# HJakeCunningham/ASVGP

Hardware: AMD Instinct MI355X
Metric: Mpoints/s per ELBO+grad step, N=10M 1D Matern-3/2 M=2048 (higher is better)
Workload: dtype f64

## Files before the change

asvgp_amd/csrc/bcr_mfma.hpp:

```cpp
#pragma once
#include "bcr.hpp"
#include "prior_plan.hpp"

namespace asvgp {

constexpr int BM_THREADS = 1024;
constexpr int BM_B = 4;
constexpr int BM_GAT = 0, BM_GBT = 16, BM_DINV = 32, BM_SD = 48, BM_CAT = 64, BM_CBT = 80, BM_W = 96, BM_DG = 100, BM_REC = 104;

__host__ __device__ inline size_t bcr_mfma_ws_doubles(long nb) { return (size_t)nb * BM_REC + 64; }
__host__ __device__ inline size_t bcr_mfma_lds_doubles(long nb) {
  return (size_t)((nb + 1) / 2 + 1) * 32 + (size_t)nb * 4 + 96 + (size_t)(BM_THREADS / 64) * 4 * 40 + (size_t)(nb / 8 + 2) * 52;
}

__device__ __forceinline__ double bm_mfma(double a, double b, double c) { return __builtin_amdgcn_mfma_f64_4x4x4f64(a, b, c, 0, 0, 0); }

__device__ __forceinline__ double bm_chol_linv(const double (&d)[10], int hi, int lo, double& dprod, int& badj) {
  double l00, i0, l10, l20, l30, l11, i1, l21, l31, l22, i2, l32, l33, i3;
  Num<double>::sqrt_inv(d[0], l00, i0);
  badj = !(d[0] > 0.0) ? 1 : 0;
  l10 = d[1] * i0; l20 = d[3] * i0; l30 = d[6] * i0;
  double s = fma(-l10, l10, d[2]);
  badj = (!(s > 0.0) && !badj) ? 2 : badj;
  Num<double>::sqrt_inv(s, l11, i1);
// ... 118 lines not shown
    const int col = n * B + cc, row = (n + 1) * B + rr;
    const bool pad = row >= M;
    const double v = bm_src_load(A, B + rr - cc, pad ? 0 : col, (long)M, 0);
    return pad ? 0.0 : v;
  };
  if ((nb & 1) && tid < 16 && !(split && sp.half == 0)) {
    const int rr = tid >> 2, cc = tid & 3;
    Dl[(size_t)((nb - 1) >> 1) * 16 + tid] = bandD(nb - 1, rr > cc ? rr : cc, rr > cc ? cc : rr);
  }
  if (split && sp.half == 0 && tid < 16) Dl[(size_t)(ht >> 1) * 16 + tid] = 0.0;
  for (int row = tid; row < nb * B; row += BM_THREADS) {
    const bool sep_left = split && sp.half == 0 && row >= ht * B && row < (ht + 1) * B;
    xs[row] = (row < M && !sep_left) ? rhs[(long)row * rhs_stride] : 0.0;
  }
  __syncthreads();
  stamp();

  constexpr int RMAXR = 4;
  for (int l = 0; l < levels; ++l) {
    const int h = 1 << l;
    const int ne = (nb > h) ? (nb - h + 2 * h - 1) / (2 * h) : 0;
    int m0, ne_h;
    level_share(l, ne, m0, ne_h);
    if (split && l == top) {
      if (sp.half == 1) {
        if (wv == 0) {
          const double v = lane < 16 ? Dl[(size_t)(ht >> 1) * 16 + lane] : (lane < 20 ? xs[ht * B + lane - 16] : 0.0);
          bm_msg_send(sp.xchg, 20, v, sp.tag | 1ull, lane);
        }
        const double mine = (r == 0 && c == 0) ? (log(ld.m) + (double)ld.e * 0.6931471805599453094) : 0.0;
        const double tot = wave_sum_dpp(mine);
        int bm = bad ? bad : 0x7fffffff;
#pragma unroll
        for (int off = 32; off > 0; off >>= 1) { const int o = __shfl_xor(bm, off, 64); bm = o < bm ? o : bm; }
        int* sbad = reinterpret_cast<int*>(red + 32);
        if (lane == 0) { red[wv] = tot; sbad[wv] = bm; }
        __syncthreads();
        if (wv == 0) {
          double sv = 0.0;
          int bmin = 0x7fffffff;
          for (int w2 = 0; w2 < BM_THREADS / 64; ++w2) { sv += red[w2]; bmin = sbad[w2] < bmin ? sbad[w2] : bmin; }
          bm_msg_send(sp.xchg + 24, 2, lane == 0 ? sv : (double)bmin, sp.tag | 2ull, lane);
        }
      } else {
        if (wv == 0) {
          double v = 0.0;
          if (!bm_msg_recv(sp.xchg, 20, v, sp.tag | 1ull, lane, sp.spin_limit)) { if (lane == 0) *sp.gave_up = 1; }
          else {
            if (lane < 16) Dl[(size_t)(ht >> 1) * 16 + lane] += v;
            else if (lane < 20) xs[ht * B + lane - 16] += v;
          }
        }
        __syncthreads();
        if (*sp.gave_up) return;
      }
      stamp();
    }
    double updb[RMAXR], ybu[RMAXR];
    int qv = q, ev = e;
    asm volatile("" : "+v"(qv), "+v"(ev));
    double sl[2][3];
    auto slab_loads = [&](int rd0) __attribute__((always_inline)) {
#pragma unroll
      for (int u = 0; u < 2; ++u) {
#pragma unroll
        for (int t3 = 0; t3 < 3; ++t3) {
          sl[u][t3] = 0.0;
          int m = (rd0 + u) * 64 + wv * 4 + qv;
          m = m0 + (m < ne_h ? m : ne_h - 1);
          const int kk = ev + 16 * t3, dd = kk >> 3, col = m * 2 * B + (kk & 7);
          const bool in = kk < 40 && col + dd < M;
          const double v = bm_src_load(A, in ? dd : 0, in ? col : 0, (long)M, 0);
          sl[u][t3] = in ? v : ((dd == 0) ? 1.0 : 0.0);
// ... 48 lines not shown
      if (act && badj && !bad) bad = i * B + badj;
      const double linv = (r >= c) ? t : 0.0;
      const double linvT = (c >= r) ? t : 0.0;
      if (act) ld.mul(dprod);
      const double ua = bm_mfma(linvT, ea, 0.0);
      const double ub = bm_mfma(linvT, eb, 0.0);
      const double zz = bm_mfma(linvT, yv, 0.0);
      const double nua = -ua, nub = -ub;
      const double da_new = bm_mfma(nua, ua, da);
      const double e_new = bm_mfma(nub, ua, 0.0);
      const double ya_new = bm_mfma(nua, zz, ya);
      updb[rd] = bm_mfma(ub, ub, 0.0);
      ybu[rd] = bm_mfma(ub, zz, 0.0);
      updb[rd] = act ? updb[rd] : 0.0;
      ybu[rd] = act ? ybu[rd] : 0.0;
      const double gat = bm_mfma(ua, linv, 0.0);
      const double gbt = bm_mfma(ub, linv, 0.0);
      const double dinv = bm_mfma(linv, linv, 0.0);
      const double w = bm_mfma(linv, zz, 0.0);
      if (act) {
        if (l >= 3) {
          double* R = Fl + (size_t)(i >> 3) * 52;
          R[e] = gat; R[16 + e] = gbt; R[32 + e] = dinv;
          if (c == 0) R[48 + r] = w;
        } else {
          double* R = rec(i);
          R[BM_GAT + e] = gat; R[BM_GBT + e] = gbt; R[BM_DINV + e] = dinv;
          if (c == 0) R[BM_W + r] = w;
        }
        Dl[(size_t)(a >> 1) * 16 + e] = da_new;
        El[(size_t)(a >> 1) * 16 + e] = e_new;
        if (c == 0) xs[a * B + r] = ya_new;
      }
    }
    bcr_lds_barrier();
#pragma unroll
    for (int rd = 0; rd < RMAXR; ++rd) {
      if (rd * 64 + wv * 4 >= ne_h) continue;
      const int ml = rd * 64 + wv * 4 + q;
      const int i = h + (m0 + ml) * 2 * h, b = i + h;
      if (ml < ne_h && b < nb) {
        Dl[(size_t)(b >> 1) * 16 + e] -= updb[rd];
        if (c == 0) xs[b * B + r] -= ybu[rd];
      }
    }
    bcr_lds_barrier();
    stamp();
  }
  if (wv == 0 && !(split && sp.half == 1)) {
    const bool act = q == 0;
    double d[10];
    int kk = 0;
#pragma unroll
    for (int rr = 0; rr < 4; ++rr)
#pragma unroll
      for (int cc = 0; cc <= rr; ++cc) { const double v = Dl[rr * 4 + cc]; d[kk++] = act ? v : ((rr == cc) ? 1.0 : 0.0); }
    const double yv = (act && c == 0) ? xs[r] : 0.0;
    double dprod;
    int badj;
    const double t = bm_chol_linv(d, hi, lo, dprod, badj);
    if (act && badj && !bad) bad = badj;
    const double linv = (r >= c) ? t : 0.0, linvT = (c >= r) ? t : 0.0;
    if (act) ld.mul(dprod);
    const double s00 = bm_mfma(linv, linv, 0.0);
    const double zz = bm_mfma(linvT, yv, 0.0);
    const double x0 = bm_mfma(linv, zz, 0.0);
    if (act) {
      rec(0)[BM_SD + e] = s00;
// ... 289 lines not shown
```

asvgp_amd/csrc/elbo.hip:

```cpp
#include <stdlib.h>
#include <time.h>
#include <string.h>

#include "bcr_pre.hpp"
#include "bcr_mfma.hpp"
#include "handle.hpp"

namespace asvgp {


struct Ws {
  double *Kuu, *dK, *P, *LK, *dLK, *LP, *SK, *dSK, *SP, *c, *alpha, *logdets, *fin, *bcrK, *bcrP;
};
static size_t bcr_ws_chain(int planes, int k, bool big) {
  long ns = 1024;
  while ((long)planes * 2 * k * k * ns * 8 + 2 * ns * k * 8 + 1024 > 150 * 1024) ns >>= 1;
  if (big) ns *= 2;
  return (size_t)planes * (7 * k * k + k) * 2 * ns + (big ? (size_t)planes * k * k * ns : 0);
}
static size_t bcr_ws_K(int k, long M) {
  size_t a = bcr_ws_chain(2, k, false), b = bcr_ws_chain(2, k, true), c = bcr_pre_ws_doubles(k, (M + k - 1) / k);
  a = a > b ? a : b;
  return (a > c ? a : c) + 64;
}
// ... 381 lines not shown
                        fin.th, fin.alpha_scale, fin.gacc, fin.ticket, fin.arrived, fin.out);
}

template <int K>
__global__ __launch_bounds__(BM_THREADS) void elbo_chains_mfma_kernel(KuuInterior ki, const double* S_static, KuuCoefs2 cf, double* Kuu, double* dK, const double* A, const double* b, int M,
                                                                      double* wsP, double* SP, double* x, double* logdets, int* info,
                                                                      double s, const double* tab, int n_rec, const int* node_rec,
                                                                      double* wsK, double* SK, double* dSK,
                                                                      unsigned long long* done_flag, unsigned long long seq,
                                                                      const unsigned long long* ready_flag, long spin_limit, FusedFin fin, const ThetaBox* box) {
  extern __shared__ double lds[];
  static_assert(K == BM_B, "matrix-core chains: bandwidth 4");
  const long E = (long)(K + 1) * M;
  const unsigned long long t_start = fin.debug_stamps ? __builtin_amdgcn_s_memrealtime() : 0ull;
  auto rstamp = [&](int slot) {
    if (fin.debug_stamps && threadIdx.x == 0 && blockIdx.x <= 2)
      logdets[(slot < 4 ? 8 + 4 * (int)blockIdx.x : 24) + slot] = (slot == 0) ? (double)(t_start & 0xffffffffull) : (double)((__builtin_amdgcn_s_memrealtime() - t_start) & 0xffffffffull);
  };
  rstamp(0);
  __shared__ int gave_up, kuu_ok;
  __shared__ double kuu_pref[4];
  if (threadIdx.x == 0) { gave_up = 0; kuu_ok = 0; }
  __syncthreads();
  double s_v = s, asc_v = fin.alpha_scale;
  ElboScalars th_v = fin.th;
  if (box) {
    if (threadIdx.x == 0) {
      long spins = 0;
      for (;;) {
        const unsigned long long got = __hip_atomic_load(&box->seq, __ATOMIC_RELAXED, __HIP_MEMORY_SCOPE_SYSTEM);
        if (got == seq) break;
        if (got == ~0ull || ++spins > spin_limit) { gave_up = 1; break; }
        __builtin_amdgcn_s_sleep(2);
      }
    }
    __syncthreads();
    if (gave_up) { if (threadIdx.x == 0) atomicExch(info + 1, -1); return; }
    s_v = box->s; asc_v = box->alpha_scale;
    th_v.v = box->v; th_v.l = box->l; th_v.s = box->s; th_v.N = box->N; th_v.Nw = box->Nw; th_v.cw = box->cw;
  }
  const double* stats = fin.stats;
  enum { LOGK, LOGP, TRKA, DTRKA, SKDK, SPDK, SKK, SPK, SPA, CC, AKA, ADKA, AAA, BA, NACC };
  double acc[NACC];
#pragma unroll
  for (int i = 0; i < NACC; ++i) acc[i] = 0.0;
  const bool isP = blockIdx.x == 0 || (fin.split && blockIdx.x == 2);
  const bool isPR = fin.split && blockIdx.x == 2;
  __shared__ double kdl[16];
  __shared__ double bnd[2 * PRIOR_BND_DIAGS * PRIOR_BND], dkb[2 * 5 * KI_DKB];
  {
    if (isP) rstamp(1);
    if (threadIdx.x == 0) {
      if (box) {
#pragma unroll
        for (int i = 0; i < 5; ++i) { kdl[i] = box->k[i]; kdl[8 + i] = box->dk[i]; }
      } else {
        kdl[0] = ki.k[0]; kdl[1] = ki.k[1]; kdl[2] = ki.k[2]; kdl[3] = ki.k[3]; kdl[4] = ki.k[4];
        kdl[8] = ki.dk[0]; kdl[9] = ki.dk[1]; kdl[10] = ki.dk[2]; kdl[11] = ki.dk[3]; kdl[12] = ki.dk[4];
      }
    }
    {
      const double* bnd_g = box ? box->bnd : reinterpret_cast<const double*>((const char*)__builtin_amdgcn_kernarg_segment_ptr() + offsetof(KuuInterior, bnd));
      const double* dkb_g = box ? box->dkb : reinterpret_cast<const double*>((const char*)__builtin_amdgcn_kernarg_segment_ptr() + offsetof(KuuInterior, dkb));
      if (threadIdx.x < 2 * PRIOR_BND_DIAGS * PRIOR_BND) bnd[threadIdx.x] = bnd_g[threadIdx.x];
      else if (threadIdx.x < 2 * PRIOR_BND_DIAGS * PRIOR_BND + 2 * 5 * KI_DKB) dkb[threadIdx.x - 2 * PRIOR_BND_DIAGS * PRIOR_BND] = dkb_g[threadIdx.x - 2 * PRIOR_BND_DIAGS * PRIOR_BND];
    }
    __syncthreads();
  }
  if (isP) {
    BmSplit bsp;
    if (fin.split) { bsp.half = isPR ? 1 : 0; bsp.xchg = fin.xchg; bsp.spin_limit = spin_limit; bsp.gave_up = &gave_up; bsp.tag = seq << 8; }
    bcr_mfma_solve<BandSumToep>(BandSumToep{A, 1.0 / s_v, (lds_cdouble_ptr)kdl, (lds_cdouble_ptr)bnd, ki.lo, ki.hi}, b, M, wsP, lds, SP, x, logdets + 2, info + 1, 1,
                                fin.debug_stamps ? (isPR ? fin.xchg + 128 : logdets + 32) : (double*)nullptr, bsp);
    rstamp(3);
    __syncthreads();
    if (gave_up) { if (threadIdx.x == 0) atomicExch(info + 1, -1); return; }
    rstamp(4);
    if (fin.finalize) {
      const double* xs_l = lds + (size_t)2 * ((((M + K - 1) / K) + 1) / 2 + 1) * 16;
      static_assert(BM_THREADS == 1024, "two columns per thread");
      int nbl = (M + K - 1) / K, lv = 0;
      while ((1 << lv) < nbl) ++lv;
      const long jsep = (long)(1 << (lv > 0 ? lv - 1 : 0)) * K;
      const long j0 = isPR ? jsep : 0, j1 = (fin.split && !isPR) ? jsep : (long)M;
      unsigned long long kw = 0ull;
      const bool kuu_reader = !isPR && (threadIdx.x >> 6) == 1;
      if (kuu_reader && (threadIdx.x & 63) <= 4)
        kw = __hip_atomic_load(reinterpret_cast<const unsigned long long*>(fin.gacc + 8) + (threadIdx.x & 63), __ATOMIC_RELAXED, __HIP_MEMORY_SCOPE_AGENT);
      double sp[2][K + 1], av[2][K + 1], bj[2];
#pragma unroll
      for (int cI = 0; cI < 2; ++cI) {
        const long j = j0 + threadIdx.x + cI * BM_THREADS, jc = j < j1 ? j : j1 - 1;
#pragma unroll
        for (int r = 0; r <= K; ++r) { sp[cI][r] = SP[(long)r * M + jc]; av[cI][r] = stats[(long)r * M + jc]; }
        bj[cI] = stats[(long)(K + 1) * M + jc];
      }
#pragma unroll
      for (int cI = 0; cI < 2; ++cI) {
        const long j = j0 + threadIdx.x + cI * BM_THREADS;
        if (j >= j1) continue;
        const bool left = j < ki.lo, right = j >= ki.hi;
        const double xj = xs_l[j];
#pragma unroll
        for (int r = 0; r <= K; ++r) {
          const long o = (long)r * M + j;
          const double w2 = (r == 0) ? 1.0 : 2.0;
          double kv = kdl[r], dkv = kdl[8 + r];
          if (left || right) {
            kv = bnd[left ? (long)r * PRIOR_BND + j : (long)(PRIOR_BND_DIAGS + r) * PRIOR_BND + (j - ki.hi)];
            if (ki.dk_tab) {
              dkv = dkb[left ? (long)r * KI_DKB + j : (long)(5 + r) * KI_DKB + (j - ki.hi)];
            } else {
              dkv = 0.0;
              for (int t = 0; t < cf.n; ++t) dkv = fma(box ? box->dc[t] : cf.dc[t], S_static[(long)t * E + o], dkv);
            }
          }
          const double xx = (j + r < M) ? w2 * xj * xs_l[j + r] : 0.0;
          acc[SPDK] = fma(w2 * sp[cI][r], dkv, acc[SPDK]);
// ... 100 lines not shown
    for (int i = 1; i < 7; ++i) v = (lane == i) ? red[i] : v;
    bm_msg_send(isPR ? box_pr : box_kuu, nmine, v, mtag | (isPR ? 5ull : 4ull), lane);
    if (threadIdx.x == 0) rstamp(2);
    return;
  }
  double kuu_v = 0.0, pr_v = 0.0;
  {
    bool ok = true;
    if (kuu_ok) kuu_v = lane < 4 ? kuu_pref[lane] : 0.0;
    else ok = bm_msg_recv(box_kuu, 4, kuu_v, mtag | 4ull, lane, spin_limit);
    if (ok && fin.split) ok = bm_msg_recv(box_pr, 7, pr_v, mtag | 5ull, lane, spin_limit);
    if (!ok) { if (lane == 0) atomicExch(info + 1, -1); return; }
  }
  {
    const int pidx[7] = {SPDK, SPK, SPA, AKA, ADKA, AAA, BA};
#pragma unroll
    for (int i = 0; i < 7; ++i) tot[pidx[i]] = red[i] + (fin.split ? __shfl(pr_v, i, 64) : 0.0);
  }
  tot[TRKA] = __shfl(kuu_v, 0, 64); tot[DTRKA] = __shfl(kuu_v, 1, 64); tot[SKDK] = __shfl(kuu_v, 2, 64); tot[SKK] = __shfl(kuu_v, 3, 64);
  if (threadIdx.x != 0) return;
#pragma unroll
  for (int i = 0; i < 14; ++i) __hip_atomic_store(fin.gacc + i, 0.0, __ATOMIC_RELAXED, __HIP_MEMORY_SCOPE_AGENT);
  {
    const double v = th_v.v, sn = th_v.s, N = th_v.N, Nw = th_v.Nw;
    const double yy = stats[(long)(K + 1) * M + M];
    const double asc = asc_v;
    tot[AKA] *= asc * asc; tot[ADKA] *= asc * asc; tot[AAA] *= asc * asc; tot[BA] *= asc;
    tot[LOGK] = __hip_atomic_load(logdets + 0, __ATOMIC_RELAXED, __HIP_MEMORY_SCOPE_AGENT);
    tot[LOGP] = __hip_atomic_load(logdets + 2, __ATOMIC_RELAXED, __HIP_MEMORY_SCOPE_AGENT);
    tot[CC] = tot[BA] / sn;
    const double two_pi = 6.283185307179586476925286766559;
    double elbo = -0.5 * N * log(two_pi * sn);
    elbo -= 0.5 * tot[LOGP];
    elbo += 0.5 * tot[LOGK];
    elbo -= 0.5 * yy / sn;
    elbo += 0.5 * tot[CC];
    elbo -= 0.5 * Nw * v / sn;
    elbo += 0.5 * tot[TRKA] / sn;
    if (th_v.cw != 0.0) elbo += th_v.cw;
    const double d_l = 0.5 * (tot[SKDK] - tot[SPDK] - tot[ADKA] + tot[DTRKA] / sn);
    const double d_v = 0.5 * (-tot[SKK] / v + tot[SPK] / v + tot[AKA] / v + tot[TRKA] / (v * sn)) - 0.5 * Nw / sn;
    const double s2 = sn * sn;
    const double d_s = -0.5 * N / sn + 0.5 * tot[SPA] / s2 + 0.5 * yy / s2 + 0.5 * tot[AAA] / s2 - tot[BA] / s2 + 0.5 * Nw * v / s2 - 0.5 * tot[TRKA] / s2;
    double* out = fin.out;
    out[0] = elbo; out[1] = d_v; out[2] = d_l; out[3] = d_s;
    out[4] = tot[LOGK]; out[5] = tot[LOGP]; out[6] = tot[TRKA]; out[7] = tot[CC];
    if (fin.mirror) {
      double* m = fin.mirror;
      const double mv[10] = {elbo, d_v, d_l, d_s, tot[LOGK], tot[LOGP], tot[TRKA], tot[CC],
                             (double)__hip_atomic_load(info, __ATOMIC_RELAXED, __HIP_MEMORY_SCOPE_AGENT),
                             (double)__hip_atomic_load(info + 1, __ATOMIC_RELAXED, __HIP_MEMORY_SCOPE_AGENT)};
      double sum = (double)fin.mirror_seq;
#pragma unroll
      for (int i = 0; i < 10; ++i) { __hip_atomic_store(m + i, mv[i], __ATOMIC_RELAXED, __HIP_MEMORY_SCOPE_SYSTEM); sum += mv[i]; }
      __hip_atomic_store(m + 11, sum, __ATOMIC_RELAXED, __HIP_MEMORY_SCOPE_SYSTEM);
      __hip_atomic_store(m + 10, (double)fin.mirror_seq, __ATOMIC_RELAXED, __HIP_MEMORY_SCOPE_SYSTEM);
    }
  }
  rstamp(2);
}

static __global__ void scale_sub_kernel(const double* __restrict__ a, const double* __restrict__ b, double* __restrict__ o,
                                 long n) {
  long i = (long)blockIdx.x * blockDim.x + threadIdx.x;
  if (i < n) o[i] = a[i] - b[i];
}
static __global__ void scale_kernel(double* __restrict__ x, double f, long n) {
  long i = (long)blockIdx.x * blockDim.x + threadIdx.x;
  if (i < n) x[i] = x[i] * f;
}

template <int K, bool TANGENT>
static int run_chains(Handle* h, const double* stats, const double* S, int kind, double v, double l, double s, long M, long D,
                      Ws w, int* info, hipStream_t st, bool& use_bcr, int part = 0, bool scale_alpha = true, FusedFin* fin = nullptr) {
  double t_enter = 0.0;
  if (debug_env().host_times) { timespec ts; clock_gettime(CLOCK_MONOTONIC, &ts); t_enter = ts.tv_sec * 1e6 + ts.tv_nsec * 1e-3; }
  KuuCoefs2 cf;
  for (int t = 0; t < ASVGP_MAX_KUU_TERMS; ++t) cf.c[t] = cf.dc[t] = 0.0;
  int rc = asvgp_matern_coeffs(kind, v, l, cf.c, cf.dc, &cf.n);
  if (rc) return rc;
  const long E = (long)(K + 1) * M;
  const double* A = stats;
  const double* b = stats ? stats + E : nullptr;
  const long nb = (M + K - 1) / K;
  const int algo = h->band_algo;
  const bool have_plan = h->plan && prior_plan_M(h->plan) == M && prior_plan_k(h->plan) == K && prior_plan_terms(h->plan) == cf.n;
  if ((algo == 3 || algo == 4) && !have_plan) { set_error("band algorithms 3 and 4 need asvgp_prior_plan_1d for this (M, k, kernel)"); return ASVGP_ERR_BAD_ARG; }
  size_t ldsK = sizeof(double) * (TANGENT ? bcr_lds_doubles<Dual, K, 0>(nb) : bcr_lds_doubles<double, K, 0>(nb));
  size_t ldsP = sizeof(double) * bcr_lds_doubles<double, K, 1>(nb);
  bool planned = have_plan && (algo == 0 || algo == 3 || algo == 4);
  size_t lds_bytes = planned ? ldsP : (ldsK > ldsP ? ldsK : ldsP);
  bool fits = lds_bytes <= 160 * 1024 - 256;
  bool big = false;
  constexpr bool HAS_BIG = (K <= 5);
  if (HAS_BIG && !fits) {
    size_t bK = sizeof(double) * (TANGENT ? bcr_lds_doubles<Dual, K, 0, true>(nb) : bcr_lds_doubles<double, K, 0, true>(nb));
    size_t bP = sizeof(double) * bcr_lds_doubles<double, K, 1, true>(nb);
    size_t bb = planned ? bP : (bK > bP ? bK : bP);
    if (bb <= 160 * 1024 - 256) { big = true; fits = true; lds_bytes = bb; }
// ... 15 lines not shown
        prior_plan_interior_kuu(h->plan, cf.c, ki.k, &ki.lo, &ki.hi, ki.bnd);
        use_mfma = ki.hi > ki.lo;
        if (use_mfma) {
          double bnd2[2 * PRIOR_BND_DIAGS * PRIOR_BND];
          long lo2 = 0, hi2 = 0;
          prior_plan_interior_kuu(h->plan, cf.dc, ki.dk, &lo2, &hi2, bnd2);
          ki.dk_tab = (ki.lo <= KI_DKB && M - ki.hi <= KI_DKB) ? 1 : 0;
          for (int sd = 0; sd < 2; ++sd)
            for (int d = 0; d <= K; ++d)
              for (int cI = 0; cI < KI_DKB; ++cI)
                ki.dkb[(sd * 5 + d) * KI_DKB + cI] = bnd2[(size_t)(sd * PRIOR_BND_DIAGS + d) * PRIOR_BND + cI];
        }
      }
    }
    if (algo == 4 && !use_mfma) {
      set_error("band algorithm 4 (matrix-core chains) needs k = 4, D = 1, M <= 2048, Toeplitz static bands and the ELBO + gradient entry point");
      return ASVGP_ERR_UNSUPPORTED;
    }
    if (h->ahead_req && !use_mfma) { set_error("launch-ahead exists for the matrix-core launch only (k = 4, D = 1, M <= 2048, planned prior chain)"); return ASVGP_ERR_UNSUPPORTED; }
    if (!use_mfma && !fits) { set_error("BCR needs %zu B of LDS", lds_bytes); return ASVGP_ERR_LDS_CAPACITY; }
    unsigned long long seq = 0;
    int slot = 0;
    double t_acq0 = 0.0, t_acq1 = 0.0;
    if (debug_env().host_times) { timespec ts; clock_gettime(CLOCK_MONOTONIC, &ts); t_acq0 = ts.tv_sec * 1e6 + ts.tv_nsec * 1e-3; }
    double* tab = handle_table_acquire(h, &seq, &slot);
    if (debug_env().host_times) { timespec ts; clock_gettime(CLOCK_MONOTONIC, &ts); t_acq1 = ts.tv_sec * 1e6 + ts.tv_nsec * 1e-3; }
    const bool gpu_fwd = h->prior_forward_gpu;
    const double* tab_k = h->tab_dev + (size_t)slot * h->slot_doubles;
    const unsigned long long* dd_ready = nullptr;
    if (gpu_fwd) {
      double* t = nullptr;
      rc = handle_prior_dd_forward(h, cf.c, cf.dc, slot, st, &t, nullptr, use_mfma ? seq : 0ull, use_mfma ? &dd_ready : nullptr);
      if (rc) return rc;
      tab_k = t;
    }
    size_t lds_pre = sizeof(double) * bcr_pre_lds_doubles(K, n_rec);
    if (lds_pre > lds_bytes) lds_bytes = lds_pre;
    FusedFin ff{};
    if (fin) { ff = *fin; ff.finalize = 1; fin->finalize = -1; }
    ff.n_helpers = (int)((M + 255) / 256 < 6 ? (M + 255) / 256 : 6);
    ff.split = 0; ff.xchg = nullptr;
    ff.assembled = reinterpret_cast<unsigned*>(w.fin + 20);
    ff.debug_no_assembly = debug_env().no_assembly;
    ff.debug_stamps = debug_env().chain_stamps;
    const long spin_limit = debug_env().spin_limit;
    if constexpr (K == BM_B) {
      if (use_mfma) {
        size_t lb = sizeof(double) * bcr_mfma_lds_doubles(nb), lk = sizeof(double) * bcr_mfma_pre_lds_doubles(nb, n_rec);
        if (lk > lb) lb = lk;
        if (sizeof(double) * FIN_LDS_DOUBLES > lb) lb = sizeof(double) * FIN_LDS_DOUBLES;
        auto kern = elbo_chains_mfma_kernel<K>;
        static size_t lds_granted[16] = {0};
        size_t& granted = lds_granted[h->device & 15];
        if (lb > granted) {
          hipError_t e = hipFuncSetAttribute(reinterpret_cast<const void*>(kern), hipFuncAttributeMaxDynamicSharedMemorySize, (int)lb);
          if (e != hipSuccess) { set_error("hipFuncSetAttribute: %s", hipGetErrorString(e)); return ASVGP_ERR_LDS_CAPACITY; }
          granted = lb;
        }
        if (h->mirror_dev) { ff.mirror = h->mirror_dev; ff.mirror_seq = ++h->mirror_seq; h->mirror_pending = ff.mirror_seq; }
        if (nb >= 128 && !debug_env().no_split) {
          ff.split = 1;
          ff.xchg = w.LP;
        }
        ff.n_helpers = 0;
        const bool plan_first = debug_env().plan_first != 0;
        const bool host_times = debug_env().host_times != 0;
        auto now_us = []() { timespec ts; clock_gettime(CLOCK_MONOTONIC, &ts); return ts.tv_sec * 1e6 + ts.tv_nsec * 1e-3; };
        const double t0 = host_times ? now_us() : 0.0;
        if (plan_first && !gpu_fwd) (void)prior_plan_eval(h->plan, cf.c, cf.dc, tab);
        const ThetaBox* box_k = nullptr;
        if (h->ahead_req) {
          if (gpu_fwd || plan_first) { set_error("launch-ahead needs the host forward pass (asvgp_set_prior_forward(h, 0))"); return ASVGP_ERR_UNSUPPORTED; }
          static_assert(sizeof(ThetaBox) <= BOX_BYTES, "theta box");
          if (!h->box_host) {
            if (hipHostMalloc(&h->box_host, BOX_BYTES * TAB_SLOTS, hipHostMallocMapped | hipHostMallocPortable | hipHostMallocCoherent) != hipSuccess ||
                hipHostGetDevicePointer(&h->box_dev, h->box_host, 0) != hipSuccess) {
              if (h->box_host) { (void)hipHostFree(h->box_host); h->box_host = nullptr; }
              set_error("launch-ahead: pinned allocation failed: %s", hipGetErrorString(hipGetLastError()));
              return ASVGP_ERR_HIP;
            }
            memset(h->box_host, 0, BOX_BYTES * TAB_SLOTS);
          }
          ThetaBox* bh = reinterpret_cast<ThetaBox*>(static_cast<char*>(h->box_host) + (size_t)slot * BOX_BYTES);
          __atomic_store_n(&bh->seq, 0ull, __ATOMIC_RELEASE);
          box_k = reinterpret_cast<const ThetaBox*>(static_cast<const char*>(h->box_dev) + (size_t)slot * BOX_BYTES);
        }
        const bool to_worker = !plan_first && !gpu_fwd && h->fwd_worker && !h->ahead_req;
        if (to_worker) {
          for (int t = 0; t < ASVGP_MAX_KUU_TERMS; ++t) { h->fwd.coef[t] = cf.c[t]; h->fwd.dcoef[t] = cf.dc[t]; }
// ... 49 lines not shown
    }
    if (scale_alpha) {
      long n = M * D;
      hipLaunchKernelGGL(scale_kernel, dim3((unsigned)((n + 255) / 256)), dim3(256), 0, st, w.alpha, 1.0 / s, n);
    }
    return check_launch("elbo chains (planned prior)");
  }
  const bool pfly = (part == 2) && use_bcr;
  if (!pfly)
    hipLaunchKernelGGL(elbo_prepare_kernel, dim3((unsigned)((E + 255) / 256)), dim3(256), 0, st, S, cf, E, A, s,
                       part == 2 ? w.LK : w.Kuu, part == 2 ? (double*)nullptr : w.dK, part == 1 ? (double*)nullptr : w.P);
  if (h->sync_on && part == 1) (void)hipEventRecord(h->evK, st);
  if (h->sync_on && part == 2) (void)hipStreamWaitEvent(st, h->evK, 0);
  if (use_bcr) {
    if (!fits) { set_error("BCR forced but needs %zu B of LDS", lds_bytes); return ASVGP_ERR_LDS_CAPACITY; }
    hipError_t e = hipFuncSetAttribute(big ? reinterpret_cast<const void*>(elbo_bcr_kernel<K, TANGENT, HAS_BIG>) : reinterpret_cast<const void*>(elbo_bcr_kernel<K, TANGENT, false>), hipFuncAttributeMaxDynamicSharedMemorySize, (int)lds_bytes);
    if (e != hipSuccess) { set_error("hipFuncSetAttribute: %s", hipGetErrorString(e)); return ASVGP_ERR_LDS_CAPACITY; }
    if (part == 1 && TANGENT) {
      if constexpr (TANGENT) {
        auto kern = big ? elbo_bcr_prior_kernel<K, HAS_BIG> : elbo_bcr_prior_kernel<K, false>;
        e = hipFuncSetAttribute(reinterpret_cast<const void*>(kern), hipFuncAttributeMaxDynamicSharedMemorySize, (int)lds_bytes);
        if (e != hipSuccess) { set_error("hipFuncSetAttribute: %s", hipGetErrorString(e)); return ASVGP_ERR_LDS_CAPACITY; }
        hipLaunchKernelGGL(kern, dim3(1), dim3(BCR_THREADS), lds_bytes, st, w.Kuu, w.dK, (int)M, w.bcrK, w.SK, w.dSK, w.logdets, info,
                           debug_env().bcr_stamps);
      }
    } else if (pfly) {
      auto kern = big ? elbo_bcr_data_kernel<K, HAS_BIG> : elbo_bcr_data_kernel<K, false>;
      e = hipFuncSetAttribute(reinterpret_cast<const void*>(kern), hipFuncAttributeMaxDynamicSharedMemorySize, (int)lds_bytes);
      if (e != hipSuccess) { set_error("hipFuncSetAttribute: %s", hipGetErrorString(e)); return ASVGP_ERR_LDS_CAPACITY; }
      hipLaunchKernelGGL(kern, dim3(1), dim3(BCR_THREADS), lds_bytes, st, w.Kuu, A, b, (int)M, w.bcrP, w.SP, w.alpha, w.logdets, info,
                         debug_env().bcr_stamps, s, (int)D, (int)(lds_bytes / sizeof(double)));
    } else {
      auto kern = big ? elbo_bcr_kernel<K, TANGENT, HAS_BIG> : elbo_bcr_kernel<K, TANGENT, false>;
      hipLaunchKernelGGL(kern, dim3(part == 0 ? 2 : 1), dim3(BCR_THREADS), lds_bytes, st, w.Kuu, w.dK,
                         w.P, b, (int)M, w.bcrK, w.bcrP, w.SK, w.dSK, w.SP, w.alpha, w.logdets, info,
                         debug_env().bcr_stamps, part == 2 ? 1 : 0, (int)D, (int)(lds_bytes / sizeof(double)));
    }
    if (part == 1) {
      if (h->sync_on) (void)hipEventRecord(h->evP, st);
      return check_launch("elbo prior chain");
    }
  } else if (D == 1) {
    hipLaunchKernelGGL((elbo_factor_kernel<K, TANGENT, true>), dim3(2), dim3(64), 0, st, w.Kuu, w.dK, w.P, w.LK, w.dLK,
                       w.LP, b, w.c, (int)M, info);
    hipLaunchKernelGGL((elbo_inverse_kernel<K, TANGENT, true>), dim3(2), dim3(64), 0, st, w.LK, w.dLK, w.LP, w.SK,
                       w.dSK, w.SP, w.c, w.alpha, (int)M);
  } else {
    hipLaunchKernelGGL((elbo_factor_kernel<K, TANGENT, false>), dim3(2), dim3(64), 0, st, w.Kuu, w.dK, w.P, w.LK,
                       w.dLK, w.LP, b, w.c, (int)M, info);
    hipLaunchKernelGGL(elbo_trsv_kernel<K>, dim3((unsigned)D), dim3(64), 0, st, w.LP, (int)M, b, w.c, D, 0, 1.0);
    hipLaunchKernelGGL((elbo_inverse_kernel<K, TANGENT, false>), dim3(2), dim3(64), 0, st, w.LK, w.dLK, w.LP, w.SK,
                       w.dSK, w.SP, w.c, w.alpha, (int)M);
    hipLaunchKernelGGL(elbo_trsv_kernel<K>, dim3((unsigned)D), dim3(64), 0, st, w.LP, (int)M, w.c, w.alpha, D, 1, 1.0);
  }
  long n = M * D;
  if (!use_bcr) hipLaunchKernelGGL(scale_kernel, dim3((unsigned)((n + 255) / 256)), dim3(256), 0, st, w.c, 1.0 / s, n);
  if (!use_bcr || scale_alpha)
    hipLaunchKernelGGL(scale_kernel, dim3((unsigned)((n + 255) / 256)), dim3(256), 0, st, w.alpha, 1.0 / s, n);
  return check_launch("elbo chains");
}

template <int K>
int ElboLauncher<K>::run(Handle* h, const double* stats, const double* S, int kind, double v, double l, double s, long N, long M, long D,
                         double* out, int* info, void* ws, hipStream_t st, int part) {
  {
    Ws w = carve(ws, M, K, D);
    bool bcr = false;
    h->mirror_pending = 0;
    ElboScalars th{v, l, s, (double)N, (double)N, 0.0};
    if (h->w_set) { th.N = h->w_npos; th.Nw = h->w_sum; th.cw = 0.5 * (double)D * h->w_sumlog; }
    const int fin_blocks = (int)((M + 255) / 256 < 64 ? (M + 255) / 256 : 64);
    static_assert(BCR_THREADS == 256, "the fused finalize shares the chain kernel's workgroup size");
    FusedFin ff{stats, th, 1.0 / s, w.fin, reinterpret_cast<unsigned*>(w.fin + 16), reinterpret_cast<unsigned*>(w.fin + 18), nullptr, out, D, 0, 0};
    int rc = run_chains<K, true>(h, stats, S, kind, v, l, s, M, D, w, info, st, bcr, part, false, part == 1 ? nullptr : &ff);
    if (rc || (part == 1)) return rc;
    if (ff.finalize < 0) return check_launch("elbo_grad_1d (fused)");
    if (h->sync_on && part == 2 && bcr && h->evP) (void)hipStreamWaitEvent(st, h->evP, 0);
    hipLaunchKernelGGL(elbo_finalize_kernel<K>, dim3(fin_blocks), dim3(256), 0, st, stats, w.Kuu, w.dK, w.LK, w.LP, w.SK,
                       w.dSK, w.SP, w.c, w.alpha, bcr ? w.logdets : (const double*)nullptr, M, K, D, th,
                       bcr ? 1.0 / s : 1.0, w.fin, reinterpret_cast<unsigned*>(w.fin + 16), out);
    return check_launch("elbo_grad_1d");
  }
}
template <int K>
int PostLauncher<K>::run(Handle* h, const double* stats, const double* S, int kind, double v, double l, double s, long M, long D,
                         double* alpha, double* W, int* info, void* ws, hipStream_t st, double* Pinv) {
  {
    Ws w = carve(ws, M, K, D);
    bool bcr = false;
    int rc = run_chains<K, false>(h, stats, S, kind, v, l, s, M, D, w, info, st, bcr);
    if (rc) return rc;
    long E = (long)(K + 1) * M;
    hipLaunchKernelGGL(scale_sub_kernel, dim3((unsigned)((E + 255) / 256)), dim3(256), 0, st, w.SP, w.SK, W, E);
    hipError_t e = hipMemcpyAsync(alpha, w.alpha, sizeof(double) * M * D, hipMemcpyDeviceToDevice, st);
    if (e == hipSuccess && Pinv) e = hipMemcpyAsync(Pinv, w.SP, sizeof(double) * E, hipMemcpyDeviceToDevice, st);
    if (e != hipSuccess) { set_error("hipMemcpyAsync: %s", hipGetErrorString(e)); return ASVGP_ERR_HIP; }
    return check_launch(Pinv ? "posterior_prepare_loo_1d" : "posterior_prepare_1d");
  }
}
// ... 434 lines not shown
```

asvgp_amd/csrc/phi_pass.hip:

```cpp
#include <stdlib.h>

#include "handle.hpp"

namespace asvgp {

constexpr int PHI_THREADS = 1024;
constexpr int PHI_CH = 32;
constexpr int PHI_MAX_BLOCKS = 256;
constexpr size_t PHI_LDS_BUDGET = 160 * 1024 - 512;

template <int K> struct FxTab {
  int g[K + 1];
  constexpr FxTab() : g{} {
    double cf[K + 1][K + 1] = {};
    for (int i = 0; i <= K; ++i)
      for (int p = 0; p <= K; ++p) cf[i][p] = piece_coef<K, 0>(i, p);
    for (int d = 0; d <= K; ++d) {
      double mx = 0.0;
      for (int i = 0; i + d <= K; ++i)
        for (int q = 0; q <= 32; ++q) {
          const double t = q / 32.0;
          double a = cf[i][K], b = cf[i + d][K];
          for (int p = K - 1; p >= 0; --p) { a = a * t + cf[i][p]; b = b * t + cf[i + d][p]; }
          if (a * b > mx) mx = a * b;
// ... 592 lines not shown
  if (avail <= 0) return 0;
  return (int)(avail / (8 * (K + 2 + (fx ? 1 : 0))));
}

template <int K, int CS>
static int launch_phi_moments_cs(Handle* h, const double* x, const double* y, long N, const double* mesh, long n_mesh, double delta,
                                 long M, double* stats, double* ws, hipStream_t st, bool regular, double step) {
  const int ncells = (int)n_mesh - 1;
  const size_t lds_bytes = mq_lds_bytes<K, CS>(M);
  if (ncells > CS || lds_bytes > PHI_LDS_BUDGET) return 1;
  long nblk = (N + 2 * MQ_THREADS - 1) / (2 * MQ_THREADS);
  const long gmax = (h->phi_blocks > 0 && h->phi_blocks < PHI_MAX_BLOCKS) ? h->phi_blocks : PHI_MAX_BLOCKS;
  const int G = (int)(nblk < 1 ? 1 : (nblk > gmax ? gmax : nblk));
  long ppb = (N + G - 1) / G;
  ppb = ((ppb + 2 * MQ_THREADS - 1) / (2 * MQ_THREADS)) * (2 * MQ_THREADS);
  int s0 = 50;
  { long c = 2; int lg = 1; while (c < ppb) { c <<= 1; ++lg; } if (62 - lg < s0) s0 = 62 - lg; }
  MqArgs a;
  a.x = x; a.y = y; a.N = N; a.mesh_g = mesh; a.n_mesh = (int)n_mesh; a.inv_delta = 1.0 / delta; a.M = (int)M; a.step = step;
  a.partials = ws;
  a.ov = ws + (size_t)PHI_MAX_BLOCKS * ((size_t)(K + 2) * M + 1);
  a.ppb = ppb; a.zero_ptr = stats; a.zero_n = (K + 2) * M + 1; a.s0 = s0;
  auto kern = regular ? phi_moment_kernel<K, CS, true> : phi_moment_kernel<K, CS, false>;
  hipError_t e = hipFuncSetAttribute(reinterpret_cast<const void*>(kern), hipFuncAttributeMaxDynamicSharedMemorySize, (int)lds_bytes);
  if (e != hipSuccess) { set_error("hipFuncSetAttribute(%zu B LDS): %s", lds_bytes, hipGetErrorString(e)); return ASVGP_ERR_LDS_CAPACITY; }
  const bool prof = h->prof_on && h->prof_n < PROF_RING && (h->prof_calls++ % h->prof_every == 0);
  if (prof) (void)hipEventRecord(h->prof_ev[h->prof_n][0], st);
  hipLaunchKernelGGL(kern, dim3((unsigned)G), dim3(MQ_THREADS), lds_bytes, st, a);
  if (prof) { (void)hipEventRecord(h->prof_ev[h->prof_n][1], st); ++h->prof_n; }
  const int E1 = (int)((K + 2) * M + 1);
  const int gsplit = G >= 64 ? 16 : (G >= 8 ? 4 : 1);
  if (h->phi_defer) {
    h->pend = Handle::PendingReduce{a.partials, G, (int)M, K, stats, true, nullptr};
    return check_launch("phi_accumulate_1d (moments, reduce deferred)");
  }
  hipLaunchKernelGGL(phi_reduce_kernel, dim3((E1 + 255) / 256, gsplit), dim3(256), 0, st, a.partials, G, (int)M, K, 0, M, 1L, 0, 1, stats, (const int*)nullptr);
  return check_launch("phi_accumulate_1d (moments)");
}

template <int K>
static int launch_phi_moments(Handle* h, const double* x, const double* y, long N, long D, const double* mesh, long n_mesh, double delta,
                              long M, double* stats, double* ws, hipStream_t st) {
  if (D != 1 || N < 1 || ((reinterpret_cast<uintptr_t>(x) | reinterpret_cast<uintptr_t>(y)) & 15) != 0) return 1;
  double step = 0.0;
  const bool regular = handle_mesh_is_linspace(h, mesh, n_mesh, st, &step, nullptr, nullptr);
  int rc = launch_phi_moments_cs<K, 512>(h, x, y, N, mesh, n_mesh, delta, M, stats, ws, st, regular, step);
  if (rc == 1) rc = launch_phi_moments_cs<K, 1024>(h, x, y, N, mesh, n_mesh, delta, M, stats, ws, st, regular, step);
  if (rc == 1) rc = launch_phi_moments_cs<K, 2048>(h, x, y, N, mesh, n_mesh, delta, M, stats, ws, st, regular, step);
// ... 36 lines not shown
  }
  if (h->n_order_seen < 8) h->order_seen[h->n_order_seen++] = Handle::OrderSeen{x, N, series};
  return series != 0;
}

template <int K, int TP, int TS>
static int launch_phi_sort_as(Handle* h, const double* x, const double* y, long N, const double* mesh, long n_mesh, double delta,
                              long M, double* stats, double* ws, hipStream_t st, double step, double m0, double m_last, double margin) {
  size_t lds_bytes = ps_lds_bytes<K, TP, TS>();
  if (ps_epilogue_bytes<K>() > lds_bytes) lds_bytes = ps_epilogue_bytes<K>();
  if (lds_bytes > 160 * 1024) return 1;
  long nblk = (N + TP * PS_THREADS - 1) / (TP * PS_THREADS);
  const long gmax = (h->phi_blocks > 0 && h->phi_blocks < PHI_MAX_BLOCKS) ? h->phi_blocks : PHI_MAX_BLOCKS;
  const int G = (int)(nblk < 1 ? 1 : (nblk > gmax ? gmax : nblk));
  long ppb = (N + G - 1) / G;
  ppb = TS ? ((ppb + 127) & ~127L) : ((ppb + 1) & ~1L);
  if (ppb > 0x3fffffffL) return 1;
  PsArgs a;
  a.x = x; a.y = y; a.N = N; a.mesh_g = mesh; a.n_mesh = (int)n_mesh; a.inv_delta = 1.0 / delta; a.M = (int)M;
  a.m0 = m0; a.m_last = m_last; a.step = step; a.smax_fast = 0.5 - margin;
  a.partials = ws; a.ppb = ppb; a.zero_ptr = stats; a.zero_n = (K + 2) * M + 1; a.stamps = nullptr; a.stamps_wave = 0;
  a.ranges = reinterpret_cast<int*>(ws + (size_t)PHI_MAX_BLOCKS * ((size_t)(K + 2) * M + 1));
  auto kern = phi_sort_kernel<K, TP, 0, 1, TS>;
  hipError_t e = hipFuncSetAttribute(reinterpret_cast<const void*>(kern), hipFuncAttributeMaxDynamicSharedMemorySize, (int)lds_bytes);
  if (e != hipSuccess) { set_error("hipFuncSetAttribute(%zu B LDS): %s", lds_bytes, hipGetErrorString(e)); return ASVGP_ERR_LDS_CAPACITY; }
  const bool prof = h->prof_on && h->prof_n < PROF_RING && (h->prof_calls++ % h->prof_every == 0);
  if (prof) (void)hipEventRecord(h->prof_ev[h->prof_n][0], st);
  hipLaunchKernelGGL(kern, dim3((unsigned)G), dim3(PS_THREADS), lds_bytes, st, a);
  if (prof) { (void)hipEventRecord(h->prof_ev[h->prof_n][1], st); ++h->prof_n; }
  h->phi_last_series = TS;
  const int E1 = (int)((K + 2) * M + 1);
  const int gsplit = G >= 64 ? 16 : (G >= 8 ? 4 : 1);
  if (h->phi_defer) {
    h->pend = Handle::PendingReduce{a.partials, G, (int)M, K, stats, true, a.ranges};
    return check_launch("phi_accumulate_1d (tile sort, reduce deferred)");
  }
  hipLaunchKernelGGL(phi_reduce_kernel, dim3((E1 + 255) / 256, gsplit), dim3(256), 0, st, a.partials, G, (int)M, K, 0, M, 1L, 0, 1, stats, (const int*)a.ranges);
  return check_launch("phi_accumulate_1d (tile sort)");
}

template <int K>
static int launch_phi_sort(Handle* h, const double* x, const double* y, long N, long D, const double* mesh, long n_mesh, double delta,
                           long M, double* stats, double* ws, hipStream_t st) {
  if (D != 1 || N < 2 || M > PS_NCELL || ((reinterpret_cast<uintptr_t>(x) | reinterpret_cast<uintptr_t>(y)) & 15) != 0) return 1;
  double step = 0.0, m0 = 0.0, m_last = 0.0;
  if (!handle_mesh_is_linspace(h, mesh, n_mesh, st, &step, &m0, &m_last)) return 1;
  const double amax = fabs(m0) > fabs(m_last) ? fabs(m0) : fabs(m_last);
  const double margin = 16.0 * 2.220446049250313e-16 * amax / delta + 1e-12;
// ... 314 lines not shown
```

Before: 133,700.

## Cache LDS attribute grants, hoist split-send out of level loop, stage scalars in LDS

Several unrelated tweaks. The phi launchers now call hipFuncSetAttribute only when the requested LDS size exceeds a cached per-device grant, which removes a host API call per step. The split BCR kernel's half-1 send/reduce path moves out of the level loop behind an early break, and a few values are passed through empty asm statements to steer register allocation. The finalize kernel keeps its theta scalars in shared memory instead of registers, and the debug_env lookup is hoisted. The static grant cache is not keyed per kernel template instantiation beyond the regular flag, so a grant could be wrongly assumed for another instantiation.

```diff
diff --git a/asvgp_amd/csrc/bcr_mfma.hpp b/asvgp_amd/csrc/bcr_mfma.hpp
--- a/asvgp_amd/csrc/bcr_mfma.hpp
+++ b/asvgp_amd/csrc/bcr_mfma.hpp
@@ -164,33 +164,17 @@
     const int ne = (nb > h) ? (nb - h + 2 * h - 1) / (2 * h) : 0;
     int m0, ne_h;
     level_share(l, ne, m0, ne_h);
+    if (split && l == top && sp.half == 1) break;
     if (split && l == top) {
-      if (sp.half == 1) {
-        if (wv == 0) {
-          const double v = lane < 16 ? Dl[(size_t)(ht >> 1) * 16 + lane] : (lane < 20 ? xs[ht * B + lane - 16] : 0.0);
-          bm_msg_send(sp.xchg, 20, v, sp.tag | 1ull, lane);
-        }
-        const double mine = (r == 0 && c == 0) ? (log(ld.m) + (double)ld.e * 0.6931471805599453094) : 0.0;
-        const double tot = wave_sum_dpp(mine);
-        int bm = bad ? bad : 0x7fffffff;
-#pragma unroll
-        for (int off = 32; off > 0; off >>= 1) { const int o = __shfl_xor(bm, off, 64); bm = o < bm ? o : bm; }
-        int* sbad = reinterpret_cast<int*>(red + 32);
-        if (lane == 0) { red[wv] = tot; sbad[wv] = bm; }
-        __syncthreads();
-        if (wv == 0) {
-          double sv = 0.0;
-          int bmin = 0x7fffffff;
-          for (int w2 = 0; w2 < BM_THREADS / 64; ++w2) { sv += red[w2]; bmin = sbad[w2] < bmin ? sbad[w2] : bmin; }
-          bm_msg_send(sp.xchg + 24, 2, lane == 0 ? sv : (double)bmin, sp.tag | 2ull, lane);
-        }
-      } else {
+      int lh = lane;
+      asm volatile("" : "+v"(lh));
+      {
         if (wv == 0) {
           double v = 0.0;
           if (!bm_msg_recv(sp.xchg, 20, v, sp.tag | 1ull, lane, sp.spin_limit)) { if (lane == 0) *sp.gave_up = 1; }
           else {
-            if (lane < 16) Dl[(size_t)(ht >> 1) * 16 + lane] += v;
-            else if (lane < 20) xs[ht * B + lane - 16] += v;
+            if (lh < 16) Dl[(size_t)(ht >> 1) * 16 + lh] += v;
+            else if (lh < 20) xs[ht * B + lh - 16] += v;
           }
         }
         __syncthreads();
@@ -285,7 +269,9 @@
         if (l >= 3) {
           double* R = Fl + (size_t)(i >> 3) * 52;
           R[e] = gat; R[16 + e] = gbt; R[32 + e] = dinv;
-          if (c == 0) R[48 + r] = w;
+          int iw = i;
+          asm volatile("" : "+v"(iw));
+          if (c == 0) (Fl + (size_t)(iw >> 3) * 52)[48 + r] = w;
         } else {
           double* R = rec(i);
           R[BM_GAT + e] = gat; R[BM_GBT + e] = gbt; R[BM_DINV + e] = dinv;
@@ -307,6 +293,32 @@
         if (c == 0) xs[b * B + r] -= ybu[rd];
       }
     }
+    bcr_lds_barrier();
+    stamp();
+  }
+  if (split && sp.half == 1) {
+    int lh = lane;
+    asm volatile("" : "+v"(lh));
+    if (wv == 0) {
+      const double v = lh < 16 ? Dl[(size_t)(ht >> 1) * 16 + lh] : (lh < 20 ? xs[ht * B + lh - 16] : 0.0);
+      bm_msg_send(sp.xchg, 20, v, sp.tag | 1ull, lane);
+    }
+    const double mine = (r == 0 && c == 0) ? (log(ld.m) + (double)ld.e * 0.6931471805599453094) : 0.0;
+    const double tot = wave_sum_dpp(mine);
+    int bm = bad ? bad : 0x7fffffff;
+#pragma unroll
+    for (int off = 32; off > 0; off >>= 1) { const int o = __shfl_xor(bm, off, 64); bm = o < bm ? o : bm; }
+    int* sbad = reinterpret_cast<int*>(red + 32);
+    if (lane == 0) { red[wv] = tot; sbad[wv] = bm; }
+    __syncthreads();
+    if (wv == 0) {
+      double sv = 0.0;
+      int bmin = 0x7fffffff;
+      for (int w2 = 0; w2 < BM_THREADS / 64; ++w2) { sv += red[w2]; bmin = sbad[w2] < bmin ? sbad[w2] : bmin; }
+      bm_msg_send(sp.xchg + 24, 2, lane == 0 ? sv : (double)bmin, sp.tag | 2ull, lane);
+    }
+    stamp();
+    bcr_lds_barrier();
     bcr_lds_barrier();
     stamp();
   }
diff --git a/asvgp_amd/csrc/elbo.hip b/asvgp_amd/csrc/elbo.hip
--- a/asvgp_amd/csrc/elbo.hip
+++ b/asvgp_amd/csrc/elbo.hip
@@ -427,8 +427,8 @@
   __shared__ double kuu_pref[4];
   if (threadIdx.x == 0) { gave_up = 0; kuu_ok = 0; }
   __syncthreads();
-  double s_v = s, asc_v = fin.alpha_scale;
-  ElboScalars th_v = fin.th;
+  __shared__ double th_l[8];
+  double s_v = s;
   if (box) {
     if (threadIdx.x == 0) {
       long spins = 0;
@@ -441,8 +441,7 @@
     }
     __syncthreads();
     if (gave_up) { if (threadIdx.x == 0) atomicExch(info + 1, -1); return; }
-    s_v = box->s; asc_v = box->alpha_scale;
-    th_v.v = box->v; th_v.l = box->l; th_v.s = box->s; th_v.N = box->N; th_v.Nw = box->Nw; th_v.cw = box->cw;
+    s_v = box->s;
   }
   const double* stats = fin.stats;
   enum { LOGK, LOGP, TRKA, DTRKA, SKDK, SPDK, SKK, SPK, SPA, CC, AKA, ADKA, AAA, BA, NACC };
@@ -457,9 +456,11 @@
     if (isP) rstamp(1);
     if (threadIdx.x == 0) {
       if (box) {
+        th_l[0] = box->v; th_l[1] = box->s; th_l[2] = box->N; th_l[3] = box->Nw; th_l[4] = box->cw; th_l[5] = box->alpha_scale;
 #pragma unroll
         for (int i = 0; i < 5; ++i) { kdl[i] = box->k[i]; kdl[8 + i] = box->dk[i]; }
       } else {
+        th_l[0] = fin.th.v; th_l[1] = fin.th.s; th_l[2] = fin.th.N; th_l[3] = fin.th.Nw; th_l[4] = fin.th.cw; th_l[5] = fin.alpha_scale;
         kdl[0] = ki.k[0]; kdl[1] = ki.k[1]; kdl[2] = ki.k[2]; kdl[3] = ki.k[3]; kdl[4] = ki.k[4];
         kdl[8] = ki.dk[0]; kdl[9] = ki.dk[1]; kdl[10] = ki.dk[2]; kdl[11] = ki.dk[3]; kdl[12] = ki.dk[4];
       }
@@ -493,12 +494,14 @@
       if (kuu_reader && (threadIdx.x & 63) <= 4)
         kw = __hip_atomic_load(reinterpret_cast<const unsigned long long*>(fin.gacc + 8) + (threadIdx.x & 63), __ATOMIC_RELAXED, __HIP_MEMORY_SCOPE_AGENT);
       double sp[2][K + 1], av[2][K + 1], bj[2];
+      const double* stats_t = stats;
+      asm volatile("" : "+s"(stats_t));
 #pragma unroll
       for (int cI = 0; cI < 2; ++cI) {
         const long j = j0 + threadIdx.x + cI * BM_THREADS, jc = j < j1 ? j : j1 - 1;
 #pragma unroll
-        for (int r = 0; r <= K; ++r) { sp[cI][r] = SP[(long)r * M + jc]; av[cI][r] = stats[(long)r * M + jc]; }
-        bj[cI] = stats[(long)(K + 1) * M + jc];
+        for (int r = 0; r <= K; ++r) { sp[cI][r] = SP[(long)r * M + jc]; av[cI][r] = stats_t[(long)r * M + jc]; }
+        bj[cI] = stats_t[(long)(K + 1) * M + jc];
       }
 #pragma unroll
       for (int cI = 0; cI < 2; ++cI) {
@@ -645,9 +648,9 @@
 #pragma unroll
   for (int i = 0; i < 14; ++i) __hip_atomic_store(fin.gacc + i, 0.0, __ATOMIC_RELAXED, __HIP_MEMORY_SCOPE_AGENT);
   {
-    const double v = th_v.v, sn = th_v.s, N = th_v.N, Nw = th_v.Nw;
+    const double v = th_l[0], sn = th_l[1], N = th_l[2], Nw = th_l[3], cw = th_l[4];
     const double yy = stats[(long)(K + 1) * M + M];
-    const double asc = asc_v;
+    const double asc = th_l[5];
     tot[AKA] *= asc * asc; tot[ADKA] *= asc * asc; tot[AAA] *= asc * asc; tot[BA] *= asc;
     tot[LOGK] = __hip_atomic_load(logdets + 0, __ATOMIC_RELAXED, __HIP_MEMORY_SCOPE_AGENT);
     tot[LOGP] = __hip_atomic_load(logdets + 2, __ATOMIC_RELAXED, __HIP_MEMORY_SCOPE_AGENT);
@@ -660,7 +663,7 @@
     elbo += 0.5 * tot[CC];
     elbo -= 0.5 * Nw * v / sn;
     elbo += 0.5 * tot[TRKA] / sn;
-    if (th_v.cw != 0.0) elbo += th_v.cw;
+    if (cw != 0.0) elbo += cw;
     const double d_l = 0.5 * (tot[SKDK] - tot[SPDK] - tot[ADKA] + tot[DTRKA] / sn);
     const double d_v = 0.5 * (-tot[SKK] / v + tot[SPK] / v + tot[AKA] / v + tot[TRKA] / (v * sn)) - 0.5 * Nw / sn;
     const double s2 = sn * sn;
@@ -696,8 +699,9 @@
 template <int K, bool TANGENT>
 static int run_chains(Handle* h, const double* stats, const double* S, int kind, double v, double l, double s, long M, long D,
                       Ws w, int* info, hipStream_t st, bool& use_bcr, int part = 0, bool scale_alpha = true, FusedFin* fin = nullptr) {
+  const DebugEnv& dbg = debug_env();
   double t_enter = 0.0;
-  if (debug_env().host_times) { timespec ts; clock_gettime(CLOCK_MONOTONIC, &ts); t_enter = ts.tv_sec * 1e6 + ts.tv_nsec * 1e-3; }
+  if (dbg.host_times) { timespec ts; clock_gettime(CLOCK_MONOTONIC, &ts); t_enter = ts.tv_sec * 1e6 + ts.tv_nsec * 1e-3; }
   KuuCoefs2 cf;
   for (int t = 0; t < ASVGP_MAX_KUU_TERMS; ++t) cf.c[t] = cf.dc[t] = 0.0;
   int rc = asvgp_matern_coeffs(kind, v, l, cf.c, cf.dc, &cf.n);
@@ -759,9 +763,9 @@
     unsigned long long seq = 0;
     int slot = 0;
     double t_acq0 = 0.0, t_acq1 = 0.0;
-    if (debug_env().host_times) { timespec ts; clock_gettime(CLOCK_MONOTONIC, &ts); t_acq0 = ts.tv_sec * 1e6 + ts.tv_nsec * 1e-3; }
+    if (dbg.host_times) { timespec ts; clock_gettime(CLOCK_MONOTONIC, &ts); t_acq0 = ts.tv_sec * 1e6 + ts.tv_nsec * 1e-3; }
     double* tab = handle_table_acquire(h, &seq, &slot);
-    if (debug_env().host_times) { timespec ts; clock_gettime(CLOCK_MONOTONIC, &ts); t_acq1 = ts.tv_sec * 1e6 + ts.tv_nsec * 1e-3; }
+    if (dbg.host_times) { timespec ts; clock_gettime(CLOCK_MONOTONIC, &ts); t_acq1 = ts.tv_sec * 1e6 + ts.tv_nsec * 1e-3; }
     const bool gpu_fwd = h->prior_forward_gpu;
     const double* tab_k = h->tab_dev + (size_t)slot * h->slot_doubles;
     const unsigned long long* dd_ready = nullptr;
@@ -778,9 +782,9 @@
     ff.n_helpers = (int)((M + 255) / 256 < 6 ? (M + 255) / 256 : 6);
     ff.split = 0; ff.xchg = nullptr;
     ff.assembled = reinterpret_cast<unsigned*>(w.fin + 20);
-    ff.debug_no_assembly = debug_env().no_assembly;
-    ff.debug_stamps = debug_env().chain_stamps;
-    const long spin_limit = debug_env().spin_limit;
+    ff.debug_no_assembly = dbg.no_assembly;
+    ff.debug_stamps = dbg.chain_stamps;
+    const long spin_limit = dbg.spin_limit;
     if constexpr (K == BM_B) {
       if (use_mfma) {
         size_t lb = sizeof(double) * bcr_mfma_lds_doubles(nb), lk = sizeof(double) * bcr_mfma_pre_lds_doubles(nb, n_rec);
@@ -795,13 +799,13 @@
           granted = lb;
         }
         if (h->mirror_dev) { ff.mirror = h->mirror_dev; ff.mirror_seq = ++h->mirror_seq; h->mirror_pending = ff.mirror_seq; }
-        if (nb >= 128 && !debug_env().no_split) {
+        if (nb >= 128 && !dbg.no_split) {
           ff.split = 1;
           ff.xchg = w.LP;
         }
         ff.n_helpers = 0;
-        const bool plan_first = debug_env().plan_first != 0;
-        const bool host_times = debug_env().host_times != 0;
+        const bool plan_first = dbg.plan_first != 0;
+        const bool host_times = dbg.host_times != 0;
         auto now_us = []() { timespec ts; clock_gettime(CLOCK_MONOTONIC, &ts); return ts.tv_sec * 1e6 + ts.tv_nsec * 1e-3; };
         const double t0 = host_times ? now_us() : 0.0;
         if (plan_first && !gpu_fwd) (void)prior_plan_eval(h->plan, cf.c, cf.dc, tab);
@@ -897,19 +901,19 @@
         e = hipFuncSetAttribute(reinterpret_cast<const void*>(kern), hipFuncAttributeMaxDynamicSharedMemorySize, (int)lds_bytes);
         if (e != hipSuccess) { set_error("hipFuncSetAttribute: %s", hipGetErrorString(e)); return ASVGP_ERR_LDS_CAPACITY; }
         hipLaunchKernelGGL(kern, dim3(1), dim3(BCR_THREADS), lds_bytes, st, w.Kuu, w.dK, (int)M, w.bcrK, w.SK, w.dSK, w.logdets, info,
-                           debug_env().bcr_stamps);
+                           dbg.bcr_stamps);
       }
     } else if (pfly) {
       auto kern = big ? elbo_bcr_data_kernel<K, HAS_BIG> : elbo_bcr_data_kernel<K, false>;
       e = hipFuncSetAttribute(reinterpret_cast<const void*>(kern), hipFuncAttributeMaxDynamicSharedMemorySize, (int)lds_bytes);
       if (e != hipSuccess) { set_error("hipFuncSetAttribute: %s", hipGetErrorString(e)); return ASVGP_ERR_LDS_CAPACITY; }
       hipLaunchKernelGGL(kern, dim3(1), dim3(BCR_THREADS), lds_bytes, st, w.Kuu, A, b, (int)M, w.bcrP, w.SP, w.alpha, w.logdets, info,
-                         debug_env().bcr_stamps, s, (int)D, (int)(lds_bytes / sizeof(double)));
+                         dbg.bcr_stamps, s, (int)D, (int)(lds_bytes / sizeof(double)));
     } else {
       auto kern = big ? elbo_bcr_kernel<K, TANGENT, HAS_BIG> : elbo_bcr_kernel<K, TANGENT, false>;
       hipLaunchKernelGGL(kern, dim3(part == 0 ? 2 : 1), dim3(BCR_THREADS), lds_bytes, st, w.Kuu, w.dK,
                          w.P, b, (int)M, w.bcrK, w.bcrP, w.SK, w.dSK, w.SP, w.alpha, w.logdets, info,
-                         debug_env().bcr_stamps, part == 2 ? 1 : 0, (int)D, (int)(lds_bytes / sizeof(double)));
+                         dbg.bcr_stamps, part == 2 ? 1 : 0, (int)D, (int)(lds_bytes / sizeof(double)));
     }
     if (part == 1) {
       if (h->sync_on) (void)hipEventRecord(h->evP, st);
@@ -949,7 +953,7 @@
     FusedFin ff{stats, th, 1.0 / s, w.fin, reinterpret_cast<unsigned*>(w.fin + 16), reinterpret_cast<unsigned*>(w.fin + 18), nullptr, out, D, 0, 0};
     int rc = run_chains<K, true>(h, stats, S, kind, v, l, s, M, D, w, info, st, bcr, part, false, part == 1 ? nullptr : &ff);
     if (rc || (part == 1)) return rc;
-    if (ff.finalize < 0) return check_launch("elbo_grad_1d (fused)");
+    if (ff.finalize < 0) return rc;
     if (h->sync_on && part == 2 && bcr && h->evP) (void)hipStreamWaitEvent(st, h->evP, 0);
     hipLaunchKernelGGL(elbo_finalize_kernel<K>, dim3(fin_blocks), dim3(256), 0, st, stats, w.Kuu, w.dK, w.LK, w.LP, w.SK,
                        w.dSK, w.SP, w.c, w.alpha, bcr ? w.logdets : (const double*)nullptr, M, K, D, th,
diff --git a/asvgp_amd/csrc/phi_pass.hip b/asvgp_amd/csrc/phi_pass.hip
--- a/asvgp_amd/csrc/phi_pass.hip
+++ b/asvgp_amd/csrc/phi_pass.hip
@@ -638,8 +638,13 @@
   a.ov = ws + (size_t)PHI_MAX_BLOCKS * ((size_t)(K + 2) * M + 1);
   a.ppb = ppb; a.zero_ptr = stats; a.zero_n = (K + 2) * M + 1; a.s0 = s0;
   auto kern = regular ? phi_moment_kernel<K, CS, true> : phi_moment_kernel<K, CS, false>;
-  hipError_t e = hipFuncSetAttribute(reinterpret_cast<const void*>(kern), hipFuncAttributeMaxDynamicSharedMemorySize, (int)lds_bytes);
-  if (e != hipSuccess) { set_error("hipFuncSetAttribute(%zu B LDS): %s", lds_bytes, hipGetErrorString(e)); return ASVGP_ERR_LDS_CAPACITY; }
+  static size_t lds_granted[2][16] = {{0}};
+  size_t& granted = lds_granted[regular ? 1 : 0][h->device & 15];
+  if (lds_bytes > granted) {
+    hipError_t e = hipFuncSetAttribute(reinterpret_cast<const void*>(kern), hipFuncAttributeMaxDynamicSharedMemorySize, (int)lds_bytes);
+    if (e != hipSuccess) { set_error("hipFuncSetAttribute(%zu B LDS): %s", lds_bytes, hipGetErrorString(e)); return ASVGP_ERR_LDS_CAPACITY; }
+    granted = lds_bytes;
+  }
   const bool prof = h->prof_on && h->prof_n < PROF_RING && (h->prof_calls++ % h->prof_every == 0);
   if (prof) (void)hipEventRecord(h->prof_ev[h->prof_n][0], st);
   hipLaunchKernelGGL(kern, dim3((unsigned)G), dim3(MQ_THREADS), lds_bytes, st, a);
@@ -722,8 +727,13 @@
   a.partials = ws; a.ppb = ppb; a.zero_ptr = stats; a.zero_n = (K + 2) * M + 1; a.stamps = nullptr; a.stamps_wave = 0;
   a.ranges = reinterpret_cast<int*>(ws + (size_t)PHI_MAX_BLOCKS * ((size_t)(K + 2) * M + 1));
   auto kern = phi_sort_kernel<K, TP, 0, 1, TS>;
-  hipError_t e = hipFuncSetAttribute(reinterpret_cast<const void*>(kern), hipFuncAttributeMaxDynamicSharedMemorySize, (int)lds_bytes);
-  if (e != hipSuccess) { set_error("hipFuncSetAttribute(%zu B LDS): %s", lds_bytes, hipGetErrorString(e)); return ASVGP_ERR_LDS_CAPACITY; }
+  static size_t lds_granted[16] = {0};
+  size_t& granted = lds_granted[h->device & 15];
+  if (lds_bytes > granted) {
+    hipError_t e = hipFuncSetAttribute(reinterpret_cast<const void*>(kern), hipFuncAttributeMaxDynamicSharedMemorySize, (int)lds_bytes);
+    if (e != hipSuccess) { set_error("hipFuncSetAttribute(%zu B LDS): %s", lds_bytes, hipGetErrorString(e)); return ASVGP_ERR_LDS_CAPACITY; }
+    granted = lds_bytes;
+  }
   const bool prof = h->prof_on && h->prof_n < PROF_RING && (h->prof_calls++ % h->prof_every == 0);
   if (prof) (void)hipEventRecord(h->prof_ev[h->prof_n][0], st);
   hipLaunchKernelGGL(kern, dim3((unsigned)G), dim3(PS_THREADS), lds_bytes, st, a);
```

Result: no change. 135,700, median of 2 (+1.6%).
